# ut-amrl/vision_slam_frontend

Measured on AMD Instinct MI355X. Metric: stereo frames/s (640x480, 2000 kp/frame), higher is better.
Workload: dtype u8

## Files before the change

vision_slam_frontend_amd/csrc/k_fast.hip:

```cpp
#include "vsf_gather.h"
#include <cstdlib>

#include "vsf_internal.h"

namespace {

typedef short v2s __attribute__((ext_vector_type(2)));
constexpr int SR = VSF_FAST_STRIP_ROWS;

struct FastArgs {
  const VsfLevel* levels;
  const uint32_t* units;
  int nunits;
  const uint8_t* img0;
  size_t img0_stride;
  int img0_pitch;
  const uint8_t* pyr;
  uint32_t pyr_bytes;
  uint32_t* cand;
  uint32_t cand_entries;
  uint16_t* rowstart;
  int threshold;
  int nms;
};

__device__ __forceinline__ uint32_t wave_shr1(uint32_t v) {
  return (uint32_t)__builtin_amdgcn_update_dpp(0, (int)v, 0x138, 0xF, 0xF, true);
}
__device__ __forceinline__ uint32_t wave_shl1(uint32_t v) {
  return (uint32_t)__builtin_amdgcn_update_dpp(0, (int)v, 0x130, 0xF, 0xF, true);
}

template <class T>
__device__ __forceinline__ T uniform_copy(const T* p) {
  static_assert(sizeof(T) % 4 == 0, "dwords");
  T out;
  const uint32_t* src = reinterpret_cast<const uint32_t*>(p);
  uint32_t* dst = reinterpret_cast<uint32_t*>(&out);
#pragma unroll
  for (size_t i = 0; i < sizeof(T) / 4; i++) dst[i] = (uint32_t)__builtin_amdgcn_readfirstlane((int)src[i]);
  return out;
}

struct RowP {
  uint32_t d;
  v2s b1, b2, b3, b4, b5, b6, b7, b8;
};

__device__ __forceinline__ v2s as_v2s(uint32_t v) { return __builtin_bit_cast(v2s, v); }
__device__ __forceinline__ uint32_t as_u32(v2s v) { return __builtin_bit_cast(uint32_t, v); }

__device__ __forceinline__ void prep_row(RowP& r) {
  const uint32_t e = r.d & 0x00FF00FFu, o = (r.d >> 8) & 0x00FF00FFu;
  const uint32_t ep = wave_shr1(e), op = wave_shr1(o);
  const uint32_t en = wave_shl1(e), on = wave_shl1(o);
  r.b1 = as_v2s(op);
  r.b2 = as_v2s(__builtin_amdgcn_alignbit(e, ep, 16));
  r.b3 = as_v2s(__builtin_amdgcn_alignbit(o, op, 16));
  r.b4 = as_v2s(e);
  r.b5 = as_v2s(o);
  r.b6 = as_v2s(__builtin_amdgcn_alignbit(en, e, 16));
  r.b7 = as_v2s(__builtin_amdgcn_alignbit(on, o, 16));
  r.b8 = as_v2s(en);
}

__device__ __forceinline__ v2s vmin(v2s a, v2s b) { return __builtin_elementwise_min(a, b); }
__device__ __forceinline__ v2s vmax(v2s a, v2s b) { return __builtin_elementwise_max(a, b); }
__device__ __forceinline__ v2s vmin3(v2s a, v2s b, v2s c) {
  v2s r;
  asm("v_pk_minimum3_f16 %0, %1, %2, %3" : "=v"(r) : "v"(a), "v"(b), "v"(c));
  return r;
}
__device__ __forceinline__ v2s vmax3(v2s a, v2s b, v2s c) {
  v2s r;
  asm("v_pk_maximum3_f16 %0, %1, %2, %3" : "=v"(r) : "v"(a), "v"(b), "v"(c));
  return r;
}
__device__ __forceinline__ v2s vsubsat(v2s a, v2s b) {
  typedef unsigned short v2us __attribute__((ext_vector_type(2)));
  return __builtin_bit_cast(v2s, __builtin_elementwise_sub_sat(__builtin_bit_cast(v2us, a), __builtin_bit_cast(v2us, b)));
}

template <bool NMS>
__device__ __forceinline__ v2s score_from_circle(const v2s (&d)[16], v2s v, v2s toff) {
  v2s E[8], G[8], F[8], H[8];
#pragma unroll
  for (int j = 0; j < 8; j++) {
    E[j] = vmin(d[2 * j + 1], d[(2 * j + 2) & 15]);
    G[j] = vmax(d[2 * j + 1], d[(2 * j + 2) & 15]);
  }
#pragma unroll
  for (int j = 0; j < 8; j++) {
    F[j] = vmin(E[j], E[(j + 1) & 7]);
    H[j] = vmax(G[j], G[(j + 1) & 7]);
  }
  v2s ta[8], tb[8];
#pragma unroll
  for (int j = 0; j < 8; j++) {
    ta[j] = vmin3(F[j], F[(j + 2) & 7], vmax(d[2 * j], d[(2 * j + 9) & 15]));
    tb[j] = vmax3(H[j], H[(j + 2) & 7], vmin(d[2 * j], d[(2 * j + 9) & 15]));
  }
  const v2s A = vmax(vmax3(vmax3(ta[0], ta[1], ta[2]), vmax3(ta[3], ta[4], ta[5]), ta[6]), ta[7]);
  const v2s Bm = vmin(vmin3(vmin3(tb[0], tb[1], tb[2]), vmin3(tb[3], tb[4], tb[5]), tb[6]), tb[7]);
  const v2s sc = vsubsat(vmax(vsubsat(A, v), vsubsat(v, Bm)), toff);
  const v2s one = {1, 1};
  return NMS ? sc : vmin(sc, one);
}

template <bool NMS>
__device__ __forceinline__ v2s score_pair0(const RowP& R0, const RowP& R1, const RowP& R2, const RowP& R3, const RowP& R4,
                                           const RowP& R5, const RowP& R6, v2s toff) {
  const v2s d[16] = {R6.b4, R6.b5, R5.b6, R4.b7, R3.b7, R2.b7, R1.b6, R0.b5, R0.b4, R0.b3, R1.b2, R2.b1, R3.b1, R4.b1, R5.b2, R6.b3};
  return score_from_circle<NMS>(d, R3.b4, toff);
}
template <bool NMS>
__device__ __forceinline__ v2s score_pair1(const RowP& R0, const RowP& R1, const RowP& R2, const RowP& R3, const RowP& R4,
                                           const RowP& R5, const RowP& R6, v2s toff) {
  const v2s d[16] = {R6.b5, R6.b6, R5.b7, R4.b8, R3.b8, R2.b8, R1.b7, R0.b6, R0.b5, R0.b4, R1.b3, R2.b2, R3.b2, R4.b2, R5.b3, R6.b4};
  return score_from_circle<NMS>(d, R3.b5, toff);
}

struct ScoreRow {
  v2s s02, s13;
  v2s h3a, h3b;
  v2s h2a, h2b;
};

__device__ __forceinline__ ScoreRow make_score_row(v2s s02, v2s s13) {
  ScoreRow o;
  o.s02 = s02;
  o.s13 = s13;
  const v2s x = as_v2s(__builtin_amdgcn_alignbit(as_u32(s13), wave_shr1(as_u32(s13)), 16));
  const v2s y = as_v2s(__builtin_amdgcn_alignbit(wave_shl1(as_u32(s02)), as_u32(s02), 16));
  o.h2a = vmax(x, s13);
  o.h2b = vmax(s02, y);
  o.h3a = vmax3(x, s13, s02);
  o.h3b = vmax3(s02, y, s13);
  return o;
}

template <bool HALF, bool NMS>
__device__ __forceinline__ void fast_march_body(const FastArgs& a, int work, int image) {
  const int lane = threadIdx.x & 63;
  const uint32_t ud = uniform_copy(a.units + work);
  const int level = (int)(ud >> 24), band = (int)((ud >> 16) & 0xFF), strip0 = (int)(ud & 0x7FFF);
  const VsfLevel L = uniform_copy(a.levels + level);
  const uint8_t* src;
  int pitch;
  if (level == 0) {
    src = a.img0 + (size_t)image * a.img0_stride;
    pitch = a.img0_pitch;
  } else {
    src = a.pyr + (size_t)image * a.pyr_bytes + L.offset;
    pitch = L.pitch;
  }
  const int t = a.threshold;
  const int offs = NMS ? max(t, 1) : t;
  const v2s toff = {(short)offs, (short)offs};
  constexpr int HL = HALF ? 32 : 64;
  const int half = HALF ? (lane >> 5) : 0, hl = lane & (HL - 1);
  const int strip = strip0 + half;
  const bool valid = strip < L.nstrips;
  const int bx0 = L.fast_a0 + VSF_FAST_BAND_COLS * band;
  const int c0 = bx0 - 4 + 4 * hl;
  const bool loadable = c0 >= 0 && c0 + 3 < pitch;
  const int ys = L.y_lo + strip * SR;
  const int nrows = valid ? min(SR, L.y_hi - ys) : 0;
  const int nrows0 = min(SR, L.y_hi - (L.y_lo + strip0 * SR));
  const int sx_lo = max(L.x_lo - 1, 3), sx_hi = min(L.x_hi + 1, L.w - 3);
  uint32_t sm02 = 0, sm13 = 0, em02 = 0, em13 = 0;
#pragma unroll
  for (int j = 0; j < 4; j++) {
    const int x = c0 + j;
    const uint32_t bit = 0xFFFFu << (16 * (j >> 1));
    const bool sc_ok = ((hl >= 1 && hl <= HL - 2) || (hl == 0 && j == 3) || (hl == HL - 1 && j == 0)) && x >= sx_lo && x < sx_hi;
    const bool em_ok = hl >= 1 && hl <= HL - 2 && x >= L.x_lo && x < L.x_hi && x < bx0 + VSF_FAST_BAND_COLS;
    if (j & 1) {
      if (sc_ok) sm13 |= bit;
      if (em_ok) em13 |= bit;
    } else {
      if (sc_ok) sm02 |= bit;
      if (em_ok) em02 |= bit;
    }
  }
  if (!valid) sm02 = sm13 = em02 = em13 = 0;
  const int unit_local = (valid ? strip : strip0) * L.nbands + band;
  uint16_t* rs = a.rowstart + ((size_t)image * a.nunits + L.unit0 + unit_local) * VSF_FAST_RS_STRIDE;
  const int seg_cap = L.seg_cap, hrow = L.h;
  uint32_t* seg0 = a.cand + (size_t)image * a.cand_entries + L.cand_offset + (size_t)(strip0 * L.nbands + band) * L.seg_cap;
  const __amdgpu_buffer_rsrc_t seg_rsrc =
      __builtin_amdgcn_make_buffer_rsrc(seg0, 0, (HALF ? L.nbands + 1 : 1) * seg_cap * 4, 0x00020000);
  const uint32_t seg_off = (HALF && half && valid) ? (uint32_t)(L.nbands * seg_cap * 4) : 0u;

  const __amdgpu_buffer_rsrc_t src_rsrc =
      __builtin_amdgcn_make_buffer_rsrc(const_cast<uint8_t*>(src), 0, pitch * hrow, 0x00020000);
  const uint32_t col_off = loadable ? (uint32_t)c0 : 0xFFFFFFF0u;
  auto load_row = [&](int q) -> uint32_t {
    const int yc = min(max(ys - 1 + q, 0), hrow - 1);
    if (HALF)
      return __builtin_amdgcn_raw_buffer_load_b32(
          src_rsrc, loadable ? __umul24((uint32_t)yc, (uint32_t)pitch) + (uint32_t)c0 : 0xFFFFFFF0u, 0u, 0);
    return __builtin_amdgcn_raw_buffer_load_b32(src_rsrc, col_off, (uint32_t)(yc * pitch), 0);
  };

  const unsigned long long scorable = __builtin_amdgcn_ballot_w64((sm02 | sm13) != 0u);
  const v2s zero2 = {0, 0};
  ScoreRow S0 = make_score_row(zero2, zero2), S1 = S0, S2 = S0;
  int count_lo = 0, count_hi = 0;
  uint32_t my_rs = 0;
  const uint32_t yx0 = ((uint32_t)ys << 12) + (uint32_t)c0 + ((uint32_t)(NMS ? offs - 1 : 0) << 24);

  auto step = [&](int q, const RowP& R0, const RowP& R1, const RowP& R2, const RowP& R3, const RowP& R4,
                  const RowP& R5, RowP& R6, const ScoreRow& S_up, const ScoreRow& S_mid, ScoreRow& S_dn) {
    prep_row(R6);
    v2s s02 = zero2, s13 = zero2;
    const int sy = ys - 1 + q;
    const bool row_ok = sy >= 3 && sy < hrow - 3;
    const uint32_t far = max(__builtin_amdgcn_sad_u8(R0.d, R3.d, 0u), __builtin_amdgcn_sad_u8(R6.d, R3.d, 0u));
    const unsigned long long want = __builtin_amdgcn_ballot_w64(far > (uint32_t)t) & scorable &
                                    (HALF ? __builtin_amdgcn_ballot_w64(row_ok) : (row_ok ? ~0ull : 0ull));
    if (want != 0ull) {
      s02 = score_pair0<NMS>(R0, R1, R2, R3, R4, R5, R6, toff);
      s13 = score_pair1<NMS>(R0, R1, R2, R3, R4, R5, R6, toff);
      s02 = as_v2s(as_u32(s02) & ((!HALF || row_ok) ? sm02 : 0u));
      s13 = as_v2s(as_u32(s13) & ((!HALF || row_ok) ? sm13 : 0u));
    }
    S_dn = make_score_row(s02, s13);
    const int r = q - 2;
    if (r >= 0 && r < nrows0) {
      if (__any((as_u32(S_mid.s02) | as_u32(S_mid.s13)) != 0)) {
        uint32_t k02, k13;
        if (NMS) {
          const v2s nb02 = vmax3(S_up.h3a, S_dn.h3a, S_mid.h2a), nb13 = vmax3(S_up.h3b, S_dn.h3b, S_mid.h2b);
          k02 = as_u32((nb02 - S_mid.s02) >> 15) & as_u32(S_mid.s02) & em02;
          k13 = as_u32((nb13 - S_mid.s13) >> 15) & as_u32(S_mid.s13) & em13;
        } else {
          k02 = as_u32(S_mid.s02) & em02;
          k13 = as_u32(S_mid.s13) & em13;
        }
        if (HALF && r >= nrows) k02 = k13 = 0;
        auto below = [](unsigned long long b, int acc) -> int {
          return (int)__builtin_amdgcn_mbcnt_hi((uint32_t)(b >> 32), __builtin_amdgcn_mbcnt_lo((uint32_t)b, (uint32_t)acc));
        };
        const uint32_t yx = yx0 + ((uint32_t)r << 12);
        if (NMS) {
          const uint32_t kk = k02 | k13;
          const bool hasA = (kk & 0xFFFFu) != 0u, hasB = (kk >> 16) != 0u;
          const unsigned long long bA = __ballot(hasA), bB = __ballot(hasB);
          if ((bA | bB) != 0ull) {
            int pos = below(bB, below(bA, half ? count_hi : count_lo));
            if (HALF) pos -= half ? __popc((uint32_t)bA) + __popc((uint32_t)bB) : 0;
            const uint32_t eA = (kk << 24) + yx + ((k13 & 0xFFFFu) != 0u ? 1u : 0u);
            const uint32_t eB = ((kk & 0xFFFF0000u) << 8) + yx + 2u + ((k13 >> 16) != 0u ? 1u : 0u);
            const int posB = pos + (hasA ? 1 : 0);
            if (hasA && (!HALF || pos < seg_cap)) __builtin_amdgcn_raw_buffer_store_b32(eA, seg_rsrc, seg_off + 4u * (uint32_t)pos, 0, 0);
            if (hasB && (!HALF || posB < seg_cap)) __builtin_amdgcn_raw_buffer_store_b32(eB, seg_rsrc, seg_off + 4u * (uint32_t)posB, 0, 0);
            if (HALF) {
              count_lo += __popc((uint32_t)bA) + __popc((uint32_t)bB);
              count_hi += __popc((uint32_t)(bA >> 32)) + __popc((uint32_t)(bB >> 32));
            } else {
              count_lo += __popcll(bA) + __popcll(bB);
            }
          }
        } else {
          const bool k0 = (k02 & 0xFFFFu) != 0, k1 = (k13 & 0xFFFFu) != 0, k2 = (k02 >> 16) != 0, k3 = (k13 >> 16) != 0;
          const unsigned long long b0 = __ballot(k0), b1 = __ballot(k1), b2 = __ballot(k2), b3 = __ballot(k3);
          if ((b0 | b1 | b2 | b3) != 0ull) {
            int pos = below(b3, below(b2, below(b1, below(b0, half ? count_hi : count_lo))));
            if (HALF) {
              const int lower = __popc((uint32_t)b0) + __popc((uint32_t)b1) + __popc((uint32_t)b2) + __popc((uint32_t)b3);
              pos -= half ? lower : 0;
            }
            if (k0) {
              if (!HALF || pos < seg_cap) __builtin_amdgcn_raw_buffer_store_b32(yx, seg_rsrc, seg_off + 4u * (uint32_t)pos, 0, 0);
              ++pos;
            }
            if (k1) {
              if (!HALF || pos < seg_cap) __builtin_amdgcn_raw_buffer_store_b32(yx + 1, seg_rsrc, seg_off + 4u * (uint32_t)pos, 0, 0);
              ++pos;
            }
            if (k2) {
              if (!HALF || pos < seg_cap) __builtin_amdgcn_raw_buffer_store_b32(yx + 2, seg_rsrc, seg_off + 4u * (uint32_t)pos, 0, 0);
              ++pos;
            }
            if (k3) {
              if (!HALF || pos < seg_cap) __builtin_amdgcn_raw_buffer_store_b32(yx + 3, seg_rsrc, seg_off + 4u * (uint32_t)pos, 0, 0);
            }
            if (HALF) {
              count_lo += __popcll(b0 & 0xFFFFFFFFull) + __popcll(b1 & 0xFFFFFFFFull) + __popcll(b2 & 0xFFFFFFFFull) +
                          __popcll(b3 & 0xFFFFFFFFull);
              count_hi += __popcll(b0 >> 32) + __popcll(b1 >> 32) + __popcll(b2 >> 32) + __popcll(b3 >> 32);
            } else {
              count_lo += __popcll(b0) + __popcll(b1) + __popcll(b2) + __popcll(b3);
            }
          }
        }
      }
      if (r + 1 < SR) {
        asm("s_mov_b32 m0, %2\n\ts_nop 0\n\tv_writelane_b32 %0, %1, m0" : "+v"(my_rs) : "s"(min(count_lo, seg_cap)), "s"(r + 1));
        if (HALF)
          asm("s_mov_b32 m0, %2\n\ts_nop 0\n\tv_writelane_b32 %0, %1, m0" : "+v"(my_rs) : "s"(min(count_hi, seg_cap)), "s"(32 + r + 1));
      }
    }
  };

  RowP A0, A1, A2, A3, A4, A5, A6, A7, A8;
  A0.d = load_row(-3), A1.d = load_row(-2), A2.d = load_row(-1), A3.d = load_row(0), A4.d = load_row(1), A5.d = load_row(2),
  A6.d = load_row(3), A7.d = load_row(4);
  prep_row(A0), prep_row(A1), prep_row(A2), prep_row(A3), prep_row(A4), prep_row(A5);
  const int qe = nrows0 + 1;
#define VSF_FAST_STEP(j, r0, r1, r2, r3, r4, r5, r6, ld, su, sm, sd) \
  if (q + (j) > qe) break;                                             \
  ld.d = load_row(q + (j) + 5);                                        \
  step(q + (j), r0, r1, r2, r3, r4, r5, r6, su, sm, sd);
  for (int q = 0;; q += 9) {
    VSF_FAST_STEP(0, A0, A1, A2, A3, A4, A5, A6, A8, S0, S1, S2)
    VSF_FAST_STEP(1, A1, A2, A3, A4, A5, A6, A7, A0, S1, S2, S0)
    VSF_FAST_STEP(2, A2, A3, A4, A5, A6, A7, A8, A1, S2, S0, S1)
    VSF_FAST_STEP(3, A3, A4, A5, A6, A7, A8, A0, A2, S0, S1, S2)
    VSF_FAST_STEP(4, A4, A5, A6, A7, A8, A0, A1, A3, S1, S2, S0)
    VSF_FAST_STEP(5, A5, A6, A7, A8, A0, A1, A2, A4, S2, S0, S1)
    VSF_FAST_STEP(6, A6, A7, A8, A0, A1, A2, A3, A5, S0, S1, S2)
    VSF_FAST_STEP(7, A7, A8, A0, A1, A2, A3, A4, A6, S1, S2, S0)
    VSF_FAST_STEP(8, A8, A0, A1, A2, A3, A4, A5, A7, S2, S0, S1)
  }
#undef VSF_FAST_STEP
  if (valid) {
    if (hl < SR) rs[hl] = (uint16_t)my_rs;
    if (hl == 0) rs[SR] = (uint16_t)min(half ? count_hi : count_lo, seg_cap);
  }
}

template <bool HALF, bool NMS>
__global__ __launch_bounds__(256) void fast_march_kernel(FastArgs a, int work0, int nwork) {
  const int item = __builtin_amdgcn_readfirstlane(blockIdx.x * 4 + (threadIdx.x >> 6));
  if (item >= nwork) return;
  fast_march_body<HALF, NMS>(a, work0 + item, blockIdx.y);
}

template <bool NMS>
__global__ __launch_bounds__(256) void fast_march_both_kernel(FastArgs a, int nfull, int nhalf) {
  const int item = __builtin_amdgcn_readfirstlane(blockIdx.x * 4 + (threadIdx.x >> 6));
  if (item >= nfull + nhalf) return;
  if (item < nfull)
    fast_march_body<false, NMS>(a, item, blockIdx.y);
  else
    fast_march_body<true, NMS>(a, item, blockIdx.y);
}

template <bool HALF, bool NMS>
__global__ __launch_bounds__(1024) void fast_march_resident_kernel(FastArgs a, int work0, int nwork, int nimages,
                                                                  uint32_t* next_cell) {
  const int total = nwork * nimages;
  while (true) {
    uint32_t r;
    asm volatile(
        "s_mov_b64 s[34:35], exec\n\t"
        "s_mov_b64 exec, 1\n\t"
        "global_atomic_add %0, %1, %2, %3 sc0\n\t"
        "s_waitcnt vmcnt(0)\n\t"
        "s_mov_b64 exec, s[34:35]"
        : "=&v"(r)
        : "v"(0u), "v"(1u), "s"(next_cell)
        : "memory", "s34", "s35");
    const uint32_t u = (uint32_t)__builtin_amdgcn_readfirstlane((int)r);
    if (u >= (uint32_t)total) break;
    const int image = (int)u / nwork, cell = (int)u - image * nwork;
    fast_march_body<HALF, NMS>(a, work0 + cell, image);
  }
}

__global__ __launch_bounds__(256) void fast_emit_kernel(const VsfLevel* __restrict__ levels,
                                                        const uint32_t* __restrict__ cand, uint32_t cand_entries,
// ... 86 lines not shown
```

vision_slam_frontend_amd/csrc/k_pyramid.hip:

```cpp
#pragma clang fp contract(off)
#include <algorithm>
#include <cmath>
#include <cstdlib>
#include <type_traits>

#include "vsf_internal.h"

namespace {


typedef unsigned short v2u16 __attribute__((ext_vector_type(2)));
struct __attribute__((packed, aligned(1))) U8B {
  uint32_t lo, hi;
};

struct ResizeArgs {
  const uint8_t* src;
  size_t src_img_stride;
  int src_pitch, sw, sh;
  uint8_t* dst;
  size_t dst_img_stride;
  int dst_pitch, dw, dh;
  double scale_x, scale_y;
  int nstrips;
};

template <int kStripRows>
__global__ __launch_bounds__(256) void resize_march_kernel(ResizeArgs a) {
  const int lane = threadIdx.x & 63;
  const int strip = __builtin_amdgcn_readfirstlane(blockIdx.x * 4 + (threadIdx.x >> 6)), band = blockIdx.z;
  if (strip >= a.nstrips) return;
  const int x4 = band * 256 + lane * 4;
  const bool active = x4 < a.dw;
  auto xtap = [&](int dx) -> VsfTap {
    float fx = (float)((dx + 0.5) * a.scale_x - 0.5);
    int sx = (int)floorf(fx);
    fx -= sx;
    if (sx < 0) fx = 0, sx = 0;
    if (sx >= a.sw - 1) fx = 0, sx = a.sw - 1;
    VsfTap t;
    t.i0 = (uint16_t)sx;
    t.i1 = (uint16_t)min(sx + 1, a.sw - 1);
    t.c0 = (int16_t)__float2int_rn((1.f - fx) * 2048);
    t.c1 = (int16_t)__float2int_rn(fx * 2048);
    return t;
  };
  auto ytap = [&](int dy) -> VsfTap {
    float fy = (float)((dy + 0.5) * a.scale_y - 0.5);
    const int sy = (int)floorf(fy);
    fy -= sy;
    VsfTap t;
    t.i0 = (uint16_t)min(max(sy, 0), a.sh - 1);
    t.i1 = (uint16_t)min(max(sy + 1, 0), a.sh - 1);
    t.c0 = (int16_t)__float2int_rn((1.f - fy) * 2048);
    t.c1 = (int16_t)__float2int_rn(fy * 2048);
    return t;
  };
  const VsfTap t0 = xtap(min(x4 + 0, a.dw - 1)), t1 = xtap(min(x4 + 1, a.dw - 1)), t2 = xtap(min(x4 + 2, a.dw - 1)),
               t3 = xtap(min(x4 + 3, a.dw - 1));
  const uint32_t base = (uint32_t)min((int)t0.i0, a.sw - 8);
  auto selector = [&](const VsfTap& t) -> uint32_t {
    return (t.i0 - base) | 0x0C000C00u | ((t.i1 - base) << 16);
  };
  auto weights = [](const VsfTap& t) -> uint32_t { return (uint32_t)(uint16_t)t.c0 | ((uint32_t)(uint16_t)t.c1 << 16); };
  const uint32_t s0 = selector(t0), s1 = selector(t1), s2 = selector(t2), s3 = selector(t3);
  const uint32_t q0 = weights(t0), q1 = weights(t1), q2 = weights(t2), q3 = weights(t3);
  const uint8_t* S = a.src + (size_t)blockIdx.y * a.src_img_stride;
  uint8_t* D = a.dst + (size_t)blockIdx.y * a.dst_img_stride;

  struct H4 {
    uint32_t a, b, c, d;
  };
  auto hpass = [&](const U8B& v) -> H4 {
    H4 h;
    h.a = __builtin_amdgcn_udot2(__builtin_bit_cast(v2u16, __builtin_amdgcn_perm(v.hi, v.lo, s0)),
                                 __builtin_bit_cast(v2u16, q0), 0u, false);
    h.b = __builtin_amdgcn_udot2(__builtin_bit_cast(v2u16, __builtin_amdgcn_perm(v.hi, v.lo, s1)),
                                 __builtin_bit_cast(v2u16, q1), 0u, false);
    h.c = __builtin_amdgcn_udot2(__builtin_bit_cast(v2u16, __builtin_amdgcn_perm(v.hi, v.lo, s2)),
                                 __builtin_bit_cast(v2u16, q2), 0u, false);
    h.d = __builtin_amdgcn_udot2(__builtin_bit_cast(v2u16, __builtin_amdgcn_perm(v.hi, v.lo, s3)),
                                 __builtin_bit_cast(v2u16, q3), 0u, false);
    return h;
  };
  const int ys = strip * kStripRows;
  const VsfTap tyl = ytap(min(ys + (lane & (kStripRows - 1)), a.dh - 1));
  const uint32_t ty_rows = (uint32_t)tyl.i0 | ((uint32_t)tyl.i1 << 16);
  const uint32_t ty_wts = (uint32_t)(uint16_t)tyl.c0 | ((uint32_t)(uint16_t)tyl.c1 << 16);
  uint32_t wts[kStripRows];
  U8B v0[kStripRows], v1[kStripRows];
#pragma unroll
  for (int r = 0; r < kStripRows; r++) {
    const uint32_t rows = __builtin_amdgcn_readlane(ty_rows, r);
    wts[r] = __builtin_amdgcn_readlane(ty_wts, r);
    const uint8_t* r0 = S + (size_t)((rows & 0xFFFFu) * (uint32_t)a.src_pitch);
    const uint8_t* r1 = S + (size_t)((rows >> 16) * (uint32_t)a.src_pitch);
    v0[r] = *reinterpret_cast<const U8B*>(r0 + base);
    v1[r] = *reinterpret_cast<const U8B*>(r1 + base);
  }
#pragma unroll
  for (int r = 0; r < kStripRows; r++) {
    const H4 h0 = hpass(v0[r]), h1 = hpass(v1[r]);
    const uint32_t b0 = (wts[r] & 0xFFFFu) << 12, b1 = (wts[r] >> 16) << 12;
    auto mulhi24 = [](uint32_t x, uint32_t y) -> uint32_t {
      return (uint32_t)(((uint64_t)(x & 0xFFFFFFu) * (uint64_t)(y & 0xFFFFFFu)) >> 32);
    };
    auto vpass = [&](uint32_t u0, uint32_t u1) -> uint32_t {
      return (mulhi24(b0, u0 & 0xFFFFF0u) + mulhi24(b1, u1 & 0xFFFFF0u) + 2u) >> 2;
    };
    const uint32_t out = vpass(h0.a, h1.a) | (vpass(h0.b, h1.b) << 8) | (vpass(h0.c, h1.c) << 16) |
                         (vpass(h0.d, h1.d) << 24);
    uint8_t* drow = D + (size_t)((uint32_t)min(ys + r, a.dh - 1) * (uint32_t)a.dst_pitch);
    if (active) *reinterpret_cast<uint32_t*>(drow + (uint32_t)x4) = out;
  }
}

struct StripX {
  uint32_t s0, s1, s2, s3, q0, q1, q2, q3, base;
  int x4;
  bool active;
};
template <int R>
struct StripRows {
  U8B v[R + 2];
  uint32_t ty_i0, ty_wts;
};

__device__ __forceinline__ StripX strip_setup(const ResizeArgs& a, int band) {
  const int lane = threadIdx.x & 63;
  StripX c;
  c.x4 = band * 256 + lane * 4;
  c.active = c.x4 < a.dw;
  auto xtap = [&](int dx) -> VsfTap {
    float fx = (float)((dx + 0.5) * a.scale_x - 0.5);
    int sx = (int)floorf(fx);
    fx -= sx;
    if (sx < 0) fx = 0, sx = 0;
    if (sx >= a.sw - 1) fx = 0, sx = a.sw - 1;
    VsfTap t;
    t.i0 = (uint16_t)sx;
    t.i1 = (uint16_t)min(sx + 1, a.sw - 1);
    t.c0 = (int16_t)__float2int_rn((1.f - fx) * 2048);
    t.c1 = (int16_t)__float2int_rn(fx * 2048);
    return t;
  };
  const VsfTap t0 = xtap(min(c.x4 + 0, a.dw - 1)), t1 = xtap(min(c.x4 + 1, a.dw - 1)),
               t2 = xtap(min(c.x4 + 2, a.dw - 1)), t3 = xtap(min(c.x4 + 3, a.dw - 1));
  c.base = (uint32_t)min((int)t0.i0, a.sw - 8);
  const uint32_t base = c.base;
  auto selector = [&](const VsfTap& t) -> uint32_t {
    return (t.i0 - base) | 0x0C000C00u | ((t.i1 - base) << 16);
  };
  auto weights = [](const VsfTap& t) -> uint32_t { return (uint32_t)(uint16_t)t.c0 | ((uint32_t)(uint16_t)t.c1 << 16); };
  c.s0 = selector(t0), c.s1 = selector(t1), c.s2 = selector(t2), c.s3 = selector(t3);
  c.q0 = weights(t0), c.q1 = weights(t1), c.q2 = weights(t2), c.q3 = weights(t3);
  return c;
}

using lds_u8p = __attribute__((address_space(3))) uint8_t*;
using lds_cu8p = const __attribute__((address_space(3))) uint8_t*;
__device__ __forceinline__ uint32_t ld32(const uint8_t* p) { return *reinterpret_cast<const uint32_t*>(p); }
__device__ __forceinline__ uint32_t ld32(lds_cu8p p) { return *(const __attribute__((address_space(3))) uint32_t*)p; }
__device__ __forceinline__ void st32(uint8_t* p, uint32_t v) { *reinterpret_cast<uint32_t*>(p) = v; }
__device__ __forceinline__ void st32(lds_u8p p, uint32_t v) { *(__attribute__((address_space(3))) uint32_t*)p = v; }

__device__ __forceinline__ int ytap_row(const ResizeArgs& a, int y) {
  const int dy = min(y, a.dh - 1);
  const float fy = (float)((dy + 0.5) * a.scale_y - 0.5);
  return min(max((int)floorf(fy), 0), a.sh - 1);
}

template <int R, bool ALIGNED = false, class SP = const uint8_t*>
__device__ __forceinline__ void strip_issue_from(const ResizeArgs& a, const StripX& c, SP S, int ys,
                                                 StripRows<R>& o) {
  const int lane = threadIdx.x & 63;
  {
    const int dy = min(ys + (lane & (R - 1)), a.dh - 1);
    float fy = (float)((dy + 0.5) * a.scale_y - 0.5);
    const int sy = (int)floorf(fy);
    fy -= sy;
    o.ty_i0 = (uint32_t)min(max(sy, 0), a.sh - 1);
    o.ty_wts = (uint32_t)__float2int_rn((1.f - fy) * 2048) | ((uint32_t)__float2int_rn(fy * 2048) << 16);
  }
  const uint32_t first = __builtin_amdgcn_readlane(o.ty_i0, 0);
#pragma unroll
  for (int k = 0; k < R + 2; k++) {
    const SP row = S + (min(first + (uint32_t)k, (uint32_t)(a.sh - 1)) * (uint32_t)a.src_pitch);
    if constexpr (ALIGNED) {
      const uint32_t b0 = c.base & ~3u;
      const uint32_t d0 = ld32(row + b0), d1 = ld32(row + b0 + 4u), d2 = ld32(row + min(b0 + 8u, (uint32_t)a.src_pitch - 4u));
      o.v[k].lo = __builtin_amdgcn_alignbyte(d1, d0, c.base & 3u);
      o.v[k].hi = __builtin_amdgcn_alignbyte(d2, d1, c.base & 3u);
    } else {
      o.v[k] = *reinterpret_cast<const U8B*>((const uint8_t*)row + c.base);
    }
  }
}

template <int R>
__device__ __forceinline__ void strip_issue(const ResizeArgs& a, const StripX& c, int image, int strip, StripRows<R>& o) {
  strip_issue_from<R>(a, c, a.src + (size_t)image * a.src_img_stride, strip * R, o);
}

template <int R, class LP = uint8_t*>
__device__ __forceinline__ void strip_finish(const ResizeArgs& a, const StripX& c, int image, int ys, int yend,
                                             const StripRows<R>& in, LP lcopy = nullptr, bool to_lds = false) {
  uint8_t* D = a.dst + (size_t)image * a.dst_img_stride;
  const uint32_t first = __builtin_amdgcn_readlane(in.ty_i0, 0);
  struct H4 {
    uint32_t a, b, c, d;
  };
  H4 H[R + 2];
#pragma unroll
  for (int k = 0; k < R + 2; k++) {
    auto hsum = [&](uint32_t sel, uint32_t q) -> uint32_t {
      return __builtin_amdgcn_udot2(__builtin_bit_cast(v2u16, __builtin_amdgcn_perm(in.v[k].hi, in.v[k].lo, sel)),
                                    __builtin_bit_cast(v2u16, q), 0u, false) & 0xFFFFF0u;
    };
    H[k].a = hsum(c.s0, c.q0);
    H[k].b = hsum(c.s1, c.q1);
    H[k].c = hsum(c.s2, c.q2);
    H[k].d = hsum(c.s3, c.q3);
  }
  auto mulhi24 = [](uint32_t x, uint32_t y) -> uint32_t {
    return (uint32_t)(((uint64_t)(x & 0xFFFFFFu) * (uint64_t)(y & 0xFFFFFFu)) >> 32);
  };
#pragma unroll
  for (int r = 0; r < R; r++) {
    if (ys + r >= yend) break;
    const uint32_t wts = __builtin_amdgcn_readlane(in.ty_wts, r);
    const uint32_t b0 = (wts & 0xFFFFu) << 12, b1 = (wts >> 16) << 12;
    const bool skip = __builtin_amdgcn_readlane(in.ty_i0, r) != first + (uint32_t)r;
    auto vrow = [&](const H4& h0, const H4& h1) -> uint32_t {
      const uint32_t ta = mulhi24(b0, h0.a) + mulhi24(b1, h1.a) + 2u, tb = mulhi24(b0, h0.b) + mulhi24(b1, h1.b) + 2u;
      const uint32_t tc = mulhi24(b0, h0.c) + mulhi24(b1, h1.c) + 2u, td = mulhi24(b0, h0.d) + mulhi24(b1, h1.d) + 2u;
      const v2u16 lo = __builtin_bit_cast(v2u16, ta | (tb << 16)) >> (v2u16){2, 2};
      const v2u16 hi = __builtin_bit_cast(v2u16, tc | (td << 16)) >> (v2u16){2, 2};
      return __builtin_amdgcn_perm(__builtin_bit_cast(uint32_t, hi), __builtin_bit_cast(uint32_t, lo), 0x06040200u);
    };
    uint8_t* drow = D + (size_t)((uint32_t)(ys + r) * (uint32_t)a.dst_pitch);
    const LP lrow = lcopy + (uint32_t)(ys + r) * (uint32_t)a.dst_pitch;
    if (skip) {
      const uint32_t out = vrow(H[r + 1], H[r + 2]);
      if (c.active) *reinterpret_cast<uint32_t*>(drow + (uint32_t)c.x4) = out;
      if (to_lds && c.active) st32(lrow + (uint32_t)c.x4, out);
      asm volatile("" ::: "memory");
    } else {
      const uint32_t out = vrow(H[r], H[r + 1]);
      if (c.active) *reinterpret_cast<uint32_t*>(drow + (uint32_t)c.x4) = out;
      if (to_lds && c.active) st32(lrow + (uint32_t)c.x4, out);
    }
  }
}

template <int R>
__device__ __forceinline__ void resize_strip_unit(const ResizeArgs& a, int image, int strip, int band) {
  const StripX c = strip_setup(a, band);
  StripRows<R> rows;
  strip_issue<R>(a, c, image, strip, rows);
  strip_finish<R>(a, c, image, strip * R, a.dh, rows);
}

template <int R>
__global__ __launch_bounds__(256) void resize_strip_kernel(ResizeArgs a) {
  const int strip = __builtin_amdgcn_readfirstlane(blockIdx.x * 4 + (threadIdx.x >> 6));
  if (strip >= a.nstrips) return;
  resize_strip_unit<R>(a, blockIdx.y, strip, blockIdx.z);
}

constexpr int kTailLdsBytes = 61440;

struct PyramidArgs {
  const VsfLevel* levels;
  const uint8_t* img0;
  size_t img0_stride;
  int img0_pitch;
  uint8_t* pyr;
  uint32_t pyr_bytes;
  int l_begin, nlevels;
};

__device__ __forceinline__ ResizeArgs tail_level_args(const PyramidArgs& p, int l) {
  const VsfLevel L = p.levels[l];
  const VsfLevel P = p.levels[l - 1];
  ResizeArgs a;
  a.src = p.pyr + P.offset;
  a.src_img_stride = (size_t)p.pyr_bytes;
  a.src_pitch = P.pitch;
  a.sw = P.w;
  a.sh = P.h;
  a.dst = p.pyr + L.offset;
  a.dst_img_stride = (size_t)p.pyr_bytes;
  a.dst_pitch = L.pitch;
  a.dw = L.w;
  a.dh = L.h;
  a.scale_x = __builtin_bit_cast(double, ((unsigned long long)L.rscale_x[1] << 32) | L.rscale_x[0]);
  a.scale_y = __builtin_bit_cast(double, ((unsigned long long)L.rscale_y[1] << 32) | L.rscale_y[0]);
  a.nstrips = (L.h + 7) / 8;
  return a;
}

__global__ __launch_bounds__(1024) void pyramid_image_kernel(PyramidArgs p) {
  __shared__ __attribute__((aligned(16))) uint8_t lvl[2][kTailLdsBytes];
  __shared__ uint32_t xs[2][10][64];
  const int image = blockIdx.x;
  const int lane = threadIdx.x & 63;
  const int wave = __builtin_amdgcn_readfirstlane(threadIdx.x >> 6);
  auto publish = [&](int l) {
    const ResizeArgs a = tail_level_args(p, l);
    const StripX c = strip_setup(a, 0);
    uint32_t(*o)[64] = xs[l & 1];
    o[0][lane] = c.s0, o[1][lane] = c.s1, o[2][lane] = c.s2, o[3][lane] = c.s3;
    o[4][lane] = c.q0, o[5][lane] = c.q1, o[6][lane] = c.q2, o[7][lane] = c.q3;
    o[8][lane] = c.base;
  };
  if (wave == 0) publish(p.l_begin);
  __syncthreads();
  for (int l = p.l_begin; l < p.nlevels; l++) {
    const ResizeArgs a = tail_level_args(p, l);
    StripX c;
    {
      const uint32_t(*o)[64] = xs[l & 1];
      c.s0 = o[0][lane], c.s1 = o[1][lane], c.s2 = o[2][lane], c.s3 = o[3][lane];
      c.q0 = o[4][lane], c.q1 = o[5][lane], c.q2 = o[6][lane], c.q3 = o[7][lane];
      c.base = o[8][lane];
      c.x4 = lane * 4;
      c.active = c.x4 < a.dw;
    }
    const bool from_lds = l > p.l_begin;
    uint8_t* lcopy = (l + 1 < p.nlevels) ? lvl[(l - p.l_begin) & 1] : nullptr;
    const uint8_t* lsrc = lvl[(l - p.l_begin + 1) & 1];
    const uint8_t* gsrc = a.src + (size_t)image * a.src_img_stride;
    for (int strip = wave; strip < a.nstrips; strip += 16) {
      StripRows<8> rows;
      if (from_lds)
        strip_issue_from<8, true>(a, c, lsrc, strip * 8, rows);
      else
        strip_issue_from<8>(a, c, gsrc, strip * 8, rows);
      strip_finish<8>(a, c, image, strip * 8, a.dh, rows, lcopy, lcopy != nullptr);
    }
    if (wave == 0 && l + 1 < p.nlevels) publish(l + 1);
    __syncthreads();
  }
}

constexpr int kSlabMaxLevels = 32;
constexpr int kSlabBands = 3;
constexpr size_t kSlabTapBytes = sizeof(uint32_t) * 2 * kSlabBands * 9 * 64;
constexpr size_t kSlabFixedBytes = kSlabTapBytes + 2 * kSlabMaxLevels * sizeof(int) + (kSlabMaxLevels + 1) * sizeof(VsfLevel);

struct SlabArgs {
  PyramidArgs p;
  int la, lb;
  int nslabs;
  uint32_t cap;
  int32_t* status;
};

__device__ __forceinline__ ResizeArgs slab_level_args(const PyramidArgs& p, int l, const VsfLevel& L, const VsfLevel& P) {
  ResizeArgs a;
  if (l >= 2) {
    a.src = p.pyr + P.offset;
    a.src_img_stride = (size_t)p.pyr_bytes;
    a.src_pitch = P.pitch;
  } else {
    a.src = p.img0;
    a.src_img_stride = p.img0_stride;
    a.src_pitch = p.img0_pitch;
  }
  a.sw = P.w;
  a.sh = P.h;
  a.dst = p.pyr + L.offset;
  a.dst_img_stride = (size_t)p.pyr_bytes;
  a.dst_pitch = L.pitch;
  a.dw = L.w;
  a.dh = L.h;
  a.scale_x = __builtin_bit_cast(double, ((unsigned long long)L.rscale_x[1] << 32) | L.rscale_x[0]);
  a.scale_y = __builtin_bit_cast(double, ((unsigned long long)L.rscale_y[1] << 32) | L.rscale_y[0]);
  a.nstrips = (L.h + 7) / 8;
  return a;
}

__global__ __launch_bounds__(1024) void pyramid_slab_kernel(SlabArgs q) {
  extern __shared__ __attribute__((aligned(16))) uint8_t smem[];
  const lds_u8p buf0 = (lds_u8p)smem, buf1 = buf0 + q.cap;
  uint32_t(*xs)[kSlabBands][9][64] = reinterpret_cast<uint32_t(*)[kSlabBands][9][64]>(smem + 2 * (size_t)q.cap);
  int* s_lo = reinterpret_cast<int*>(smem + 2 * (size_t)q.cap + kSlabTapBytes);
  int* s_hi = s_lo + kSlabMaxLevels;
  VsfLevel* s_lev = reinterpret_cast<VsfLevel*>(s_hi + kSlabMaxLevels);
  const int image = blockIdx.y, slab = blockIdx.x;
// ... 47 lines not shown
    const ResizeArgs a = level_args(l);
    const int j = l - q.la;
    if (wave >= 16 - kSlabBands && l + 1 < q.lb) publish(l + 1);
    const int ylo = s_lo[j], yhi = s_hi[j];
    const int nb = (a.dw + 255) >> 8;
    const bool from_lds = j > 0;
    const bool to_lds = l + 1 < q.lb;
    const lds_u8p lcopy = ((j & 1) ? buf1 : buf0) - (uint32_t)ylo * (uint32_t)a.dst_pitch;
    const lds_cu8p lsrc = ((j & 1) ? buf0 : buf1) - (uint32_t)(from_lds ? s_lo[j - 1] : 0) * (uint32_t)a.src_pitch;
    const uint8_t* gsrc = a.src + (size_t)image * a.src_img_stride;
    auto run = [&](auto rows_tag) {
      constexpr int R = decltype(rows_tag)::value;
      const int nunits = ((yhi - ylo + R - 1) / R) * nb;
      for (int u = wave; u < nunits; u += 16) {
        const int st = u / nb, band = u - st * nb;
        StripX c;
        {
          const uint32_t(*o)[64] = xs[l & 1][band];
          c.s0 = o[0][lane], c.s1 = o[1][lane], c.s2 = o[2][lane], c.s3 = o[3][lane];
          c.q0 = o[4][lane], c.q1 = o[5][lane], c.q2 = o[6][lane], c.q3 = o[7][lane];
          c.base = o[8][lane];
          c.x4 = band * 256 + lane * 4;
          c.active = c.x4 < a.dw;
        }
        const int ys = ylo + st * R;
        StripRows<R> rows;
        if (from_lds)
          strip_issue_from<R, true, lds_cu8p>(a, c, lsrc, ys, rows);
        else
          strip_issue_from<R>(a, c, gsrc, ys, rows);
        strip_finish<R, lds_u8p>(a, c, image, ys, yhi, rows, lcopy, to_lds);
      }
    };
    if (((yhi - ylo + 1) >> 1) * nb <= 16 - kSlabBands)
      run(std::integral_constant<int, 2>{});
    else if (((yhi - ylo + 3) >> 2) * nb <= 16 - kSlabBands)
      run(std::integral_constant<int, 4>{});
    else
      run(std::integral_constant<int, 8>{});
    __syncthreads();
  }
}

size_t slab_chain_bytes(const VsfLevel* lv, int la, int lb, int nslabs) {
  long rows = (lv[lb - 1].h + nslabs - 1) / nslabs + 1;
  size_t need = 0;
  for (int l = lb - 1; l > la; l--) {
    const double sy = 1. / ((double)lv[l].h / lv[l - 1].h);
    rows = std::min<long>((long)std::floor((double)rows * sy) + 4, lv[l - 1].h);
    need = std::max(need, (size_t)rows * (size_t)lv[l - 1].pitch);
  }
  return need;
}

}

hipError_t vsf_prepare_pyramid_kernels(int lds_limit) {
  if (lds_limit < 160 * 1024 - 2048) return hipSuccess;
  return hipFuncSetAttribute(reinterpret_cast<const void*>(pyramid_slab_kernel), hipFuncAttributeMaxDynamicSharedMemorySize,
                             160 * 1024 - 2048);
}

void vsf_launch_pyramid(const VsfDev& d, const VsfGeom& g, const VsfLevel* h_levels, const VsfImages& im,
                        hipStream_t s, const VsfSideStream* side) {
  int l_tail = g.nlevels;
  const int few_max = d.tune ? d.tune->pyramid_few : 16;
  const bool few = side && im.n <= few_max;
  if (few && g.nlevels > 1) {
    bool ok = true;
    for (int l = 1; l < g.nlevels; l++) ok = ok && h_levels[l].resize_any8 && h_levels[l].w <= 256 * kSlabBands;
    const int chain_env = d.tune ? d.tune->pyramid_chain : 8;
    const int lds_limit = d.tune ? d.tune->lds_limit : 160 * 1024;
    if (ok && chain_env > 0 && lds_limit >= 160 * 1024 - 2048) {
      const size_t fixed = kSlabFixedBytes;
      const size_t budget = 144 * 1024;
      for (int la = 1; la < g.nlevels;) {
        int lb = std::min({la + chain_env, la + kSlabMaxLevels, g.nlevels});
        const int rows_env = d.tune ? std::max(1, d.tune->pyramid_rows) : 6;
        int nslabs = std::max(1, std::min(64, h_levels[lb - 1].h / rows_env));
        size_t need = slab_chain_bytes(h_levels, la, lb, nslabs);
        while (2 * need + fixed > budget && (nslabs < 64 || lb > la + 1)) {
          if (nslabs < 64)
            nslabs = std::min(64, nslabs * 2);
          else
            --lb;
          need = slab_chain_bytes(h_levels, la, lb, nslabs);
        }
        SlabArgs q;
        q.p.levels = d.levels;
        q.p.img0 = im.base;
        q.p.img0_stride = im.image_stride;
        q.p.img0_pitch = (int)im.row_stride;
        q.p.pyr = d.pyr;
        q.p.pyr_bytes = g.pyr_bytes;
        q.p.l_begin = la;
        q.p.nlevels = lb;
        q.la = la;
        q.lb = lb;
        q.nslabs = nslabs;
        q.cap = (uint32_t)((need + 255) & ~(size_t)255);
        q.status = d.status;
        hipLaunchKernelGGL(pyramid_slab_kernel, dim3(nslabs, im.n), dim3(1024), 2 * (size_t)q.cap + fixed, s, q);
        la = lb;
      }
      return;
    }
  }
  if (side && (im.n >= 64 || few || (d.tune && d.tune->pyramid_tail_min > 0 && im.n >= d.tune->pyramid_tail_min))) {
    static int ncu = 0;
    if (ncu == 0) {
      int dev = 0;
      hipDeviceProp_t prop;
      if (hipGetDevice(&dev) == hipSuccess && hipGetDeviceProperties(&prop, dev) == hipSuccess) ncu = prop.multiProcessorCount;
      if (ncu <= 0) ncu = 256;
    }
    const int rounds = (im.n + ncu - 1) / ncu;
    const int tail_min = d.tune ? d.tune->pyramid_tail_min : 0;
    if (few || 4 * im.n >= 3 * rounds * ncu || (tail_min > 0 && im.n >= tail_min)) {
      while (l_tail > 2 && h_levels[l_tail - 1].w <= 256 && h_levels[l_tail - 1].resize_rows >= 8 &&
             h_levels[l_tail - 1].pitch * h_levels[l_tail - 1].h + 16 <= kTailLdsBytes)
        --l_tail;
      if (g.nlevels - l_tail < 4) l_tail = g.nlevels;
    }
  }
  const int nchains = (side && side->n > 0 && im.n >= 2) ? 2 : 1;
  hipStream_t st[VSF_SIDE_STREAMS + 1] = {s};
  for (int c = 1; c < nchains; c++) st[c] = side->stream[c - 1];
  if (nchains > 1) {
    vsf_note(hipEventRecord(side->fork, s));
    for (int c = 1; c < nchains; c++) vsf_note(hipStreamWaitEvent(st[c], side->fork, 0));
  }
  for (int l = 1; l < l_tail; l++) {
    const VsfLevel& L = h_levels[l];
    const VsfLevel& P = h_levels[l - 1];
    for (int c = 0; c < nchains; c++) {
      const int i0 = (int)((long)im.n * c / nchains), n = (int)((long)im.n * (c + 1) / nchains) - i0;
      ResizeArgs a;
      a.src = (l == 1) ? im.base + (size_t)i0 * im.image_stride : d.pyr + (size_t)i0 * g.pyr_bytes + P.offset;
      a.src_img_stride = (l == 1) ? im.image_stride : (size_t)g.pyr_bytes;
      a.src_pitch = (l == 1) ? (int)im.row_stride : P.pitch;
      a.sw = P.w;
      a.sh = P.h;
      a.dst = d.pyr + (size_t)i0 * g.pyr_bytes + L.offset;
      a.dst_img_stride = (size_t)g.pyr_bytes;
      a.dst_pitch = L.pitch;
      a.dw = L.w;
      a.dh = L.h;
      a.scale_x = 1. / ((double)L.w / P.w);
      a.scale_y = 1. / ((double)L.h / P.h);
      const int nbands = (L.w + 255) / 256;
      const bool large = (long)L.w * L.h * n >= 4000000;
      const dim3 block(256);
      if (L.resize_rows >= 8) {
        const int R = (large && L.resize_rows >= 16) ? 16 : 8;
        a.nstrips = (L.h + R - 1) / R;
        const dim3 grid((a.nstrips + 3) / 4, n, nbands);
        if (R == 16)
          hipLaunchKernelGGL(resize_strip_kernel<16>, grid, block, 0, st[c], a);
        else
          hipLaunchKernelGGL(resize_strip_kernel<8>, grid, block, 0, st[c], a);
        continue;
      }
      const int rows = large ? 8 : 4;
      a.nstrips = (L.h + rows - 1) / rows;
      if (large)
        hipLaunchKernelGGL(resize_march_kernel<8>, dim3((a.nstrips + 3) / 4, n, nbands), dim3(256), 0, st[c], a);
      else
        hipLaunchKernelGGL(resize_march_kernel<4>, dim3((a.nstrips + 3) / 4, n, nbands), dim3(256), 0, st[c], a);
    }
  }
  for (int c = 1; c < nchains; c++) {
    vsf_note(hipEventRecord(side->join[c - 1], st[c]));
    vsf_note(hipStreamWaitEvent(s, side->join[c - 1], 0));
  }
  if (l_tail < g.nlevels) {
    PyramidArgs p;
    p.levels = d.levels;
    p.img0 = im.base;
    p.img0_stride = im.image_stride;
    p.img0_pitch = (int)im.row_stride;
    p.pyr = d.pyr;
    p.pyr_bytes = g.pyr_bytes;
    p.l_begin = l_tail;
    p.nlevels = g.nlevels;
    hipLaunchKernelGGL(pyramid_image_kernel, dim3(im.n), dim3(1024), 0, s, p);
  }
}
```

vision_slam_frontend_amd/csrc/vsf_geometry.hip:

```cpp
#include <algorithm>
#include <cfloat>
#include <climits>
#include <cmath>
#include <cstdio>
#include <cstring>
#include <new>
#include <vector>

#include "vsf_ctx.h"

using namespace vsfi;

namespace {

inline int cvRoundD(double v) { return (int)std::nearbyint(v); }
inline int cvRoundF(float v) { return (int)std::nearbyintf(v); }
inline int cvFloorD(double v) {
  const int i = cvRoundD(v);
  return i - ((float)(v - i) < 0);
}
inline int cvCeilD(double v) {
  const int i = cvRoundD(v);
  return i + ((float)(i - v) < 0);
}
// ... 75 lines not shown
    const int nbands = (L.w + 63) / 64, npairs = (nbands + 1) / 2;
    for (int b = 0; b < 2 * npairs; b++)
      for (int op = 0; op < 4; op++) {
        const int tile = 2 * b + (op >> 1);
        const int first = 32 * tile - 16 + 32 * (op & 1);
        for (int lane = 0; lane < 64; lane++) {
          const int n = lane & 31, h = lane >> 5, x = 32 * tile + n;
          int8_t wgt[16] = {0};
          if (x < L.w)
            for (int j = 0; j < 7; j++) {
              const int c = reflect101_host(x + j - 3, L.w) - (first + 16 * h);
              if (c >= 0 && c < 16) wgt[c] = (int8_t)(wgt[c] + k[j]);
            }
          uint4 v;
          memcpy(&v, wgt, 16);
          G->blur_tcol.push_back(v);
        }
      }
    const int nsteps = (L.h + VSF_BLUR_MMA_ROWS - 1) / VSF_BLUR_MMA_ROWS, ndsteps = (nsteps + 1) / 2;
    for (int pass = 0; pass < 2; pass++) {
      const int per_unit = pass == 0 ? VSF_BLUR_MMA_STEPS : VSF_BLUR_MMA_STEPS_SMALL;
      std::vector<uint32_t>& units = pass == 0 ? G->blur_mma_units : G->blur_mma_units_small;
      const int nstrips = (ndsteps + per_unit - 1) / per_unit;
      for (int st = 0; st < nstrips; st++) {
        const int s0 = (int)((long long)ndsteps * st / nstrips), s1 = (int)((long long)ndsteps * (st + 1) / nstrips);
        for (int b = 0; b < npairs; b++)
          units.push_back(((uint32_t)l << 24) | ((uint32_t)b << 16) | ((uint32_t)s0 << 8) | (uint32_t)(s1 - s0));
      }
    }
  }
  G->blur_tv.clear();
  for (int op = 0; op < 4; op++)
    for (int lane = 0; lane < 64; lane++) {
      const int n = lane & 31, h = lane >> 5, s = op & 1;
      uint16_t e[8];
      for (int j = 0; j < 8; j++) {
        const int row = 16 * s + 8 * (j >> 2) + 4 * h + (j & 3), d = row - n;
        const int tap = (n < VSF_BLUR_MMA_ROWS && d >= 0 && d < 7) ? k[d] : 0;
        e[j] = f16_bits_of_small_int(op >= 2 ? tap * 256 : tap);
      }
      uint4 v;
      memcpy(&v, e, 16);
      G->blur_tv.push_back(v);
    }
}

bool build_geometry(const vsf_params& p, bool orb, bool nms, Geometry* out) {
  Geometry& G = *out;
  const int nlevels = orb ? p.nlevels : 1;
  const int border = orb ? std::max(p.edge_threshold, 3) : 3;
  G.levels.assign(nlevels, VsfLevel{});
  G.g.nlevels = nlevels;
  G.g.width = p.width;
  G.g.height = p.height;
  const double scale_factor = (double)p.scale_factor;
  std::vector<int> nfeat(nlevels, 0);
  if (orb) {
    const float factor = (float)(1.0 / scale_factor);
    float nd = p.nfeatures * (1 - factor) / (1 - (float)std::pow((double)factor, (double)nlevels));
    int sum = 0;
    for (int l = 0; l < nlevels - 1; l++) {
      nfeat[l] = cvRoundF(nd);
      sum += nfeat[l];
      nd *= factor;
    }
    nfeat[nlevels - 1] = std::max(p.nfeatures - sum, 0);
  }
  uint32_t offset = 0;
  uint64_t pixels = 0;
  int max_w = 0;
  for (int l = 0; l < nlevels; l++) {
    VsfLevel& L = G.levels[l];
    L.scale = orb ? (float)std::pow(scale_factor, (double)(l - p.first_level)) : 1.f;
    L.w = cvRoundF(p.width / L.scale);
    L.h = cvRoundF(p.height / L.scale);
    if (L.w < 8 || L.h < 1 || L.w > 4095 || L.h > 4095) return false;
    L.pitch = align_up(L.w, 64);
    L.offset = offset;
    offset += (uint32_t)align_up(L.pitch * align_up(L.h, 8), 256);
    L.nfeatures = nfeat[l];
    pixels += (uint64_t)L.w * L.h;
    max_w = std::max(max_w, L.w);
    if (L.w <= 2 * border || L.h <= 2 * border) {
      L.x_lo = L.x_hi = L.y_lo = L.y_hi = border;
    } else {
      L.x_lo = border;
      L.x_hi = L.w - border;
      L.y_lo = border;
      L.y_hi = L.h - border;
    }
    L.blur_vec_end = p.blur_sse2 ? (L.w - L.w % 4) : 0;
  }
  G.g.pyr_bytes = offset;
  G.g.pyramid_pixels = pixels;
  uint32_t cand = 0;
  int kp_off = 0, ncells = 0;
  std::vector<uint32_t> half_items;
  for (int l = 0; l < nlevels; l++) {
    VsfLevel& L = G.levels[l];
    const int vw = L.x_hi - L.x_lo, vh = L.y_hi - L.y_lo;
    L.fast_a0 = L.x_lo & ~3;
    L.nbands = vw > 0 ? (L.x_hi - L.fast_a0 + VSF_FAST_BAND_COLS - 1) / VSF_FAST_BAND_COLS : 0;
    L.nstrips = vh > 0 && vw > 0 ? (vh + VSF_FAST_STRIP_ROWS - 1) / VSF_FAST_STRIP_ROWS : 0;
    if (L.nbands > 255 || L.nstrips > 32767) return false;
    L.unit0 = ncells;
    ncells += L.nstrips * L.nbands;
    const int last_w = L.nbands > 0 ? L.x_hi - (L.fast_a0 + VSF_FAST_BAND_COLS * (L.nbands - 1)) : 0;
    const bool half_last = L.nbands > 0 && L.nstrips >= 2 && last_w <= VSF_FAST_HALF_COLS;
    for (int s = 0; s < L.nstrips; s++)
      for (int b = 0; b < L.nbands; b++) {
        const uint32_t item = ((uint32_t)l << 24) | ((uint32_t)b << 16) | (uint32_t)s;
        if (half_last && b == L.nbands - 1) {
          if ((s & 1) == 0) half_items.push_back(item);
        } else {
          G.units.push_back(item);
        }
      }
    const int bw = std::min(VSF_FAST_BAND_COLS, std::max(vw, 1)), bh = std::min(VSF_FAST_STRIP_ROWS, std::max(vh, 1));
    L.seg_cap = nms ? ((bw + 1) / 2) * ((bh + 1) / 2) : bw * bh;
    L.seg_cap = std::max(L.seg_cap, 1);
    L.cand_offset = cand;
    cand += (uint32_t)L.seg_cap * (uint32_t)(L.nstrips * L.nbands);
    L.kp_offset = kp_off;
    L.kp_cap = 2 * L.nfeatures + 64;
    kp_off += L.kp_cap;
  }
  G.g.cand_entries = std::max(cand, 1u);
  G.g.nunits = ncells;
  G.g.nwork_full = (int)G.units.size();
  G.g.nwork_half = (int)half_items.size();
  G.units.insert(G.units.end(), half_items.begin(), half_items.end());
  if (G.units.empty()) G.units.push_back(0);
  G.g.lvlkp_entries = std::max(kp_off, 1);
  if (orb) {
    for (int l = 1; l < nlevels; l++) {
      VsfLevel& L = G.levels[l];
      const VsfLevel& P = G.levels[l - 1];
      L.xtab = (uint32_t)G.xt.size();
      L.ytab = (uint32_t)G.yt.size();
      build_taps(P.w, P.h, L.w, L.h, &G.xt, &G.yt);
      {
        const double sx = 1. / ((double)L.w / P.w), sy = 1. / ((double)L.h / P.h);
        memcpy(L.rscale_x, &sx, 8);
        memcpy(L.rscale_y, &sy, 8);
      }
      if (P.w < 8) return false;
      for (int x4 = 0; x4 < L.w; x4 += 4) {
        const int base = std::min((int)G.xt[L.xtab + x4].i0, P.w - 8);
        for (int j = 0; j < 4 && x4 + j < L.w; j++) {
          const VsfTap& t = G.xt[L.xtab + x4 + j];
          if (t.i0 < base || t.i1 - base > 7) return false;
        }
      }
      L.resize_rows = 0;
      for (int R : {16, 8, 4}) {
        bool ok = true;
        for (int ys = 0; ys < L.h && ok; ys += R) {
          const int f = G.yt[L.ytab + ys].i0;
          for (int r = 0; r < R && ys + r < L.h && ok; r++) {
            const VsfTap& t = G.yt[L.ytab + ys + r];
            const int dlt = (int)t.i0 - f - r;
            ok = (dlt == 0 || dlt == 1) && (int)t.i1 == std::min((int)t.i0 + 1, P.h - 1);
          }
        }
        if (ok) {
          L.resize_rows = R;
          break;
        }
      }
      L.resize_any8 = 1;
      for (int ys = 0; ys < L.h && L.resize_any8; ys++) {
        const int f = G.yt[L.ytab + ys].i0;
        for (int r = 0; r < 8 && ys + r < L.h && L.resize_any8; r++) {
          const VsfTap& t = G.yt[L.ytab + ys + r];
          const int dlt = (int)t.i0 - f - r;
          if (!((dlt == 0 || dlt == 1) && (int)t.i1 == std::min((int)t.i0 + 1, P.h - 1))) L.resize_any8 = 0;
        }
      }
    }
  }
  if (G.xt.empty()) G.xt.push_back(VsfTap{0, 0, 0, 0});
  if (G.yt.empty()) G.yt.push_back(VsfTap{0, 0, 0, 0});
  if (orb) {
    int k4[4];
    gaussian_taps(k4);
    const int ksum = 2 * (k4[0] + k4[1] + k4[2]) + k4[3];
    if (ksum > 257 || k4[3] > 127 || G.levels[0].w > 64 * 255 || G.levels[0].h > VSF_BLUR_MMA_ROWS * 255) return false;
    build_blur_mma_tables(&G);
  }
  if (G.blur_mma_units.empty()) G.blur_mma_units.push_back(0);
  if (G.blur_mma_units_small.empty()) G.blur_mma_units_small.push_back(0);
  if (G.blur_tcol.empty()) G.blur_tcol.push_back(make_uint4(0, 0, 0, 0));
  if (G.blur_tv.empty()) G.blur_tv.push_back(make_uint4(0, 0, 0, 0));
  return true;
}

std::vector<uint2> build_ic_table() {
  const std::vector<int> um = orb_umax(31);
  std::vector<uint2> t(4 * VSF_IC_ITEMS, make_uint2(0, 0));
  for (int s = 0; s < 4; s++)
    for (int item = 0; item < 31 * 9; item++) {
      const int r = item / 9, j = item % 9, v = r - 15, d = um[std::abs(v)];
      uint32_t wx = 0, wm = 0;
      for (int b = 0; b < 4; b++) {
        const int u = 4 * j + b - s - 15;
        if (std::abs(u) <= d) {
          wx |= (uint32_t)(u + 16) << (8 * b);
          wm |= 1u << (8 * b);
        }
      }
      t[(size_t)s * VSF_IC_ITEMS + item] = make_uint2(wx, wm);
    }
  return t;
}

void gaussian_taps(int k[4]) {
  const int n = 7;
  const double sigma = 2.0, scale2x = -0.5 / (sigma * sigma);
  float cf[7];
  double sum = 0;
  for (int i = 0; i < n; i++) {
    const double x = i - (n - 1) * 0.5;
    cf[i] = (float)std::exp(scale2x * x * x);
    sum += cf[i];
  }
  sum = 1. / sum;
  for (int i = 0; i < 4; i++) k[i] = cvRoundD((double)(float)(cf[i] * sum) * 256.0);
}

}
```

Baseline: 41210.

## Use byte perms in FAST row prep, drop SAD prefilter, add 24-row resize strips

FAST row preparation now builds its zero-extended byte pairs with v_perm instead of masks plus alignbit, and the SAD-based far-pixel ballot prefilter is removed, so scoring runs for every scorable row. In the pyramid resize, the vertical blend packs the rounding constant for both halves into one add, and a 24-row strip kernel is added for large levels whose taps allow it. Together these cut ALU work per row and raise rows per strip. Removing the prefilter makes the expensive score path run more often.

After: 41600 (median of 6 runs). About the same (+1.0%).

```diff
diff --git a/vision_slam_frontend_amd/csrc/k_fast.hip b/vision_slam_frontend_amd/csrc/k_fast.hip
--- a/vision_slam_frontend_amd/csrc/k_fast.hip
+++ b/vision_slam_frontend_amd/csrc/k_fast.hip
@@ -51,17 +51,15 @@
 __device__ __forceinline__ uint32_t as_u32(v2s v) { return __builtin_bit_cast(uint32_t, v); }
 
 __device__ __forceinline__ void prep_row(RowP& r) {
-  const uint32_t e = r.d & 0x00FF00FFu, o = (r.d >> 8) & 0x00FF00FFu;
-  const uint32_t ep = wave_shr1(e), op = wave_shr1(o);
-  const uint32_t en = wave_shl1(e), on = wave_shl1(o);
-  r.b1 = as_v2s(op);
-  r.b2 = as_v2s(__builtin_amdgcn_alignbit(e, ep, 16));
-  r.b3 = as_v2s(__builtin_amdgcn_alignbit(o, op, 16));
-  r.b4 = as_v2s(e);
-  r.b5 = as_v2s(o);
-  r.b6 = as_v2s(__builtin_amdgcn_alignbit(en, e, 16));
-  r.b7 = as_v2s(__builtin_amdgcn_alignbit(on, o, 16));
-  r.b8 = as_v2s(en);
+  const uint32_t d = r.d, p = wave_shr1(d), n = wave_shl1(d);
+  r.b1 = as_v2s(__builtin_amdgcn_perm(0u, p, 0x0C030C01u));
+  r.b2 = as_v2s(__builtin_amdgcn_perm(d, p, 0x0C040C02u));
+  r.b3 = as_v2s(__builtin_amdgcn_perm(d, p, 0x0C050C03u));
+  r.b4 = as_v2s(__builtin_amdgcn_perm(0u, d, 0x0C020C00u));
+  r.b5 = as_v2s(__builtin_amdgcn_perm(0u, d, 0x0C030C01u));
+  r.b6 = as_v2s(__builtin_amdgcn_perm(n, d, 0x0C040C02u));
+  r.b7 = as_v2s(__builtin_amdgcn_perm(n, d, 0x0C050C03u));
+  r.b8 = as_v2s(__builtin_amdgcn_perm(0u, n, 0x0C020C00u));
 }
 
 __device__ __forceinline__ v2s vmin(v2s a, v2s b) { return __builtin_elementwise_min(a, b); }
@@ -216,9 +214,7 @@
     v2s s02 = zero2, s13 = zero2;
     const int sy = ys - 1 + q;
     const bool row_ok = sy >= 3 && sy < hrow - 3;
-    const uint32_t far = max(__builtin_amdgcn_sad_u8(R0.d, R3.d, 0u), __builtin_amdgcn_sad_u8(R6.d, R3.d, 0u));
-    const unsigned long long want = __builtin_amdgcn_ballot_w64(far > (uint32_t)t) & scorable &
-                                    (HALF ? __builtin_amdgcn_ballot_w64(row_ok) : (row_ok ? ~0ull : 0ull));
+    const unsigned long long want = scorable & (HALF ? __builtin_amdgcn_ballot_w64(row_ok) : (row_ok ? ~0ull : 0ull));
     if (want != 0ull) {
       s02 = score_pair0<NMS>(R0, R1, R2, R3, R4, R5, R6, toff);
       s13 = score_pair1<NMS>(R0, R1, R2, R3, R4, R5, R6, toff);
diff --git a/vision_slam_frontend_amd/csrc/k_pyramid.hip b/vision_slam_frontend_amd/csrc/k_pyramid.hip
--- a/vision_slam_frontend_amd/csrc/k_pyramid.hip
+++ b/vision_slam_frontend_amd/csrc/k_pyramid.hip
@@ -175,7 +175,7 @@
                                                  StripRows<R>& o) {
   const int lane = threadIdx.x & 63;
   {
-    const int dy = min(ys + (lane & (R - 1)), a.dh - 1);
+    const int dy = min(ys + ((R & (R - 1)) == 0 ? (lane & (R - 1)) : lane), a.dh - 1);
     float fy = (float)((dy + 0.5) * a.scale_y - 0.5);
     const int sy = (int)floorf(fy);
     fy -= sy;
@@ -232,10 +232,10 @@
     const uint32_t b0 = (wts & 0xFFFFu) << 12, b1 = (wts >> 16) << 12;
     const bool skip = __builtin_amdgcn_readlane(in.ty_i0, r) != first + (uint32_t)r;
     auto vrow = [&](const H4& h0, const H4& h1) -> uint32_t {
-      const uint32_t ta = mulhi24(b0, h0.a) + mulhi24(b1, h1.a) + 2u, tb = mulhi24(b0, h0.b) + mulhi24(b1, h1.b) + 2u;
-      const uint32_t tc = mulhi24(b0, h0.c) + mulhi24(b1, h1.c) + 2u, td = mulhi24(b0, h0.d) + mulhi24(b1, h1.d) + 2u;
-      const v2u16 lo = __builtin_bit_cast(v2u16, ta | (tb << 16)) >> (v2u16){2, 2};
-      const v2u16 hi = __builtin_bit_cast(v2u16, tc | (td << 16)) >> (v2u16){2, 2};
+      const uint32_t tb = mulhi24(b0, h0.b) + mulhi24(b1, h1.b), td = mulhi24(b0, h0.d) + mulhi24(b1, h1.d);
+      const uint32_t ta = mulhi24(b0, h0.a) + mulhi24(b1, h1.a) + 0x20002u, tc = mulhi24(b0, h0.c) + mulhi24(b1, h1.c) + 0x20002u;
+      const v2u16 lo = __builtin_bit_cast(v2u16, (tb << 16) + ta) >> (v2u16){2, 2};
+      const v2u16 hi = __builtin_bit_cast(v2u16, (td << 16) + tc) >> (v2u16){2, 2};
       return __builtin_amdgcn_perm(__builtin_bit_cast(uint32_t, hi), __builtin_bit_cast(uint32_t, lo), 0x06040200u);
     };
     uint8_t* drow = D + (size_t)((uint32_t)(ys + r) * (uint32_t)a.dst_pitch);
@@ -589,10 +589,12 @@
       const bool large = (long)L.w * L.h * n >= 4000000;
       const dim3 block(256);
       if (L.resize_rows >= 8) {
-        const int R = (large && L.resize_rows >= 16) ? 16 : 8;
+        const int R = large ? std::min(L.resize_rows, 24) : 8;
         a.nstrips = (L.h + R - 1) / R;
         const dim3 grid((a.nstrips + 3) / 4, n, nbands);
-        if (R == 16)
+        if (R == 24)
+          hipLaunchKernelGGL(resize_strip_kernel<24>, grid, block, 0, st[c], a);
+        else if (R == 16)
           hipLaunchKernelGGL(resize_strip_kernel<16>, grid, block, 0, st[c], a);
         else
           hipLaunchKernelGGL(resize_strip_kernel<8>, grid, block, 0, st[c], a);
diff --git a/vision_slam_frontend_amd/csrc/vsf_geometry.hip b/vision_slam_frontend_amd/csrc/vsf_geometry.hip
--- a/vision_slam_frontend_amd/csrc/vsf_geometry.hip
+++ b/vision_slam_frontend_amd/csrc/vsf_geometry.hip
@@ -251,8 +251,7 @@
           if (t.i0 < base || t.i1 - base > 7) return false;
         }
       }
-      L.resize_rows = 0;
-      for (int R : {16, 8, 4}) {
+      auto strips_ok = [&](int R) {
         bool ok = true;
         for (int ys = 0; ys < L.h && ok; ys += R) {
           const int f = G.yt[L.ytab + ys].i0;
@@ -262,11 +261,16 @@
             ok = (dlt == 0 || dlt == 1) && (int)t.i1 == std::min((int)t.i0 + 1, P.h - 1);
           }
         }
-        if (ok) {
+        return ok;
+      };
+      L.resize_rows = 0;
+      for (int R : {16, 8, 4}) {
+        if (strips_ok(R)) {
           L.resize_rows = R;
           break;
         }
       }
+      if (L.resize_rows == 16 && strips_ok(24)) L.resize_rows = 24;
       L.resize_any8 = 1;
       for (int ys = 0; ys < L.h && L.resize_any8; ys++) {
         const int f = G.yt[L.ytab + ys].i0;
```
